# MLforHealth/LEMoN

Hardware: AMD Instinct MI355X
Metric: label-error scores/sec (embed+kNN), CIFAR-100 noise=0.4 (higher is better)
Workload: dtype f32-equivalent (fp16 x3 split GEMMs: hi.hi + hi.lo + lo.hi, fp32 accumulate, LayerNorms folded in: error <= fp32 GEMM x sqrt(1 + (mean/sigma)^2) <= 8.06, measured <= 1.8; everything else fp32)

## Files before the change

include/lemon_hip.h:

```cpp
#ifndef LEMON_HIP_H
#define LEMON_HIP_H

#include <stdint.h>

#ifdef __cplusplus
extern "C" {
#endif

#define LEMON_METRIC_IP 0
#define LEMON_METRIC_L2 1

#define LEMON_OK 0
#define LEMON_E_INVALID (-1)
#define LEMON_E_HIP (-2)
#define LEMON_E_NOMEM (-3)

#define LEMON_MAX_K 64
#define LEMON_MAX_K_DEEP 2048

#define LEMON_ALGO_AUTO 0
#define LEMON_ALGO_F32_MFMA 1
#define LEMON_ALGO_BF16_FILTER 2
#define LEMON_ALGO_F16_FILTER LEMON_ALGO_BF16_FILTER

// ... 59 lines not shown
int lemon_linear_f32(const float *x_dev, const float *w_dev, const float *bias_dev, const float *residual_dev,
                     int64_t m, int n, int k, float alpha, int act, float *y_dev, void *stream);

int lemon_linear_bf16x6(const uint16_t *x6_dev, const uint16_t *w6_dev, const float *bias_dev, const float *residual_dev,
                        int64_t m, int n, int k6, float alpha, int act, float *y_dev, void *stream);
int lemon_split3_f32(const float *x_dev, int64_t rows, int k, int weight, uint16_t *y6_dev, void *stream);
int lemon_layernorm_split3(const float *x_dev, const float *weight_dev, const float *bias_dev, float eps, int64_t rows,
                           int width, uint16_t *y6_dev, void *stream);
int lemon_linear_f16x3(const uint16_t *x3_dev, const uint16_t *w3_dev, const float *bias_dev, const float *residual_dev,
                       int64_t m, int n, int k3, float alpha, int act, float *y_dev, void *stream);
int lemon_split_f16x3(const float *x_dev, int64_t rows, int k, int weight, float wscale, uint16_t *y3_dev, void *stream);
int lemon_layernorm_f16x3(const float *x_dev, const float *weight_dev, const float *bias_dev, float eps, int64_t rows,
                          int width, uint16_t *y3_dev, void *stream);
int lemon_attention_f16x3(const float *qkv_dev, int64_t batch, int seq_len, int heads, int head_dim,
                          int causal, uint16_t *out3_dev, void *stream);
int lemon_attention_f16x3_varlen(const float *qkv_dev, int64_t batch, int seq_len, int heads, int head_dim,
                                 const int32_t *lengths_dev, uint16_t *out3_dev, void *stream);
int lemon_pack_weight_f16x3t(const float *w_dev, int n, int k, float wscale, uint16_t *wt_dev, void *stream);
int lemon_layernorm_f16x3t(const float *x_dev, const float *weight_dev, const float *bias_dev, float eps, int64_t rows,
                           int width, uint16_t *yt_dev, void *stream);
int lemon_linear_f16x3t(const uint16_t *at_dev, const uint16_t *wt_dev, const float *bias_dev, const float *residual_dev,
                        int64_t m, int n, int k, float alpha, int act, int out_operand, void *out_dev, void *stream);
int lemon_unpack_act_f16x3t(const uint16_t *at_dev, int64_t rows, int k, float *y_dev, void *stream);
int lemon_linear_f16x3t_ln(const uint16_t *at_dev, const uint16_t *wt_dev, const float *bias_dev, const float *residual_dev,
                           int64_t m, int n, int k, float alpha, int act, int out_operand, void *out_dev, const float *row_aff_dev,
                           const float *colsum_dev, uint16_t *emit_t_dev, float *emit_stats_dev, void *stream);
int lemon_linear_f16x3t_chain(const uint16_t *at_dev, const uint16_t *wt_dev, const float *bias_dev, const float *residual_dev,
                              const uint16_t *residual_t_dev, int64_t m, int n, int k, float alpha, float *out_dev,
                              uint16_t *emit_t_dev, float *emit_stats_dev, void *stream);
int lemon_ln_finalize(const float *partials_dev, int64_t rows, int width, float eps, float *row_aff_dev, void *stream);
int lemon_rowstats_f16x3t(const float *x_dev, float eps, int64_t rows, int width, uint16_t *yt_dev, float *row_aff_dev, void *stream);
int lemon_linear_f16x3t_set_profiling(int on);
int lemon_linear_f16x3t_set_mfma(int shape);
int lemon_linear_f16x3t_profile_read(int64_t *launches, double *kernel_ms, double *flops);
int lemon_attention_f16x3t(const float *qkv_dev, int64_t batch, int seq_len, int heads, int head_dim,
                           int causal, uint16_t *outt_dev, void *stream);
int lemon_attention_f16x3t_varlen(const float *qkv_dev, int64_t batch, int seq_len, int heads, int head_dim,
                                  const int32_t *lengths_dev, uint16_t *outt_dev, void *stream);
int lemon_linear_load_tuned(const char *path);
int lemon_linear_dump_tuned(const char *path);
int lemon_linear_set_tuning(int enabled);
int lemon_linear_stamp(int *hipblaslt_version, char *arch, int arch_len);


int lemon_index_create(int metric, int d, lemon_index_t **out);
int lemon_index_free(lemon_index_t *idx);

int lemon_index_add(lemon_index_t *idx, const float *x_dev, int64_t n, void *stream);

int64_t lemon_index_ntotal(const lemon_index_t *idx);
int lemon_index_dim(const lemon_index_t *idx);
const float *lemon_index_data(const lemon_index_t *idx);

int lemon_index_search(lemon_index_t *idx, const float *q_dev, int64_t nq, int k,
                       float *D_dev, int64_t *I_dev, void *stream);
int lemon_index_set_algo(lemon_index_t *idx, int algo);
int lemon_index_set_query_dedup(lemon_index_t *idx, int enabled);

typedef struct {
    int algo;
    int grid, block;
    int query_panel;
    int db_splits;
    int64_t nq, n;
    int d, k;
    int64_t nq_distinct;
// ... 94 lines not shown
```

lemon_amd/_lib.py:

```python
import ctypes
import os

_HERE = os.path.dirname(os.path.abspath(__file__))
SO_PATH = os.path.join(_HERE, "liblemon_hip.so")

METRIC_IP = 0
METRIC_L2 = 1
MAX_K = 64
MAX_K_DEEP = 2048
ATTENTION_MAX_SEQ = 4096
ALGO_AUTO, ALGO_F32_MFMA, ALGO_BF16_FILTER = 0, 1, 2

EXPORTS = [
    "lemon_last_error", "lemon_version", "lemon_normalize_rows", "lemon_paired_distance",
    "lemon_d1_normalized", "lemon_class_confidence", "lemon_paired_metric", "lemon_preprocess_u8", "lemon_preprocess_u8_f16x3t", "lemon_preprocess_ragged", "lemon_attention_f32", "lemon_attention_set_f16", "lemon_attention_set_stream_min", "lemon_attention_set_head_dims", "lemon_attention_get_head_dims", "lemon_attention_split3", "lemon_attention_f32_varlen", "lemon_attention_split3_varlen", "lemon_attention_f16x3_varlen", "lemon_attention_f16x3t_varlen", "lemon_layernorm_f32", "lemon_vision_tokens_ln", "lemon_text_tokens", "lemon_linear_f32", "lemon_linear_bf16x6", "lemon_split3_f32", "lemon_layernorm_split3", "lemon_linear_f16x3", "lemon_pack_weight_f16x3t", "lemon_layernorm_f16x3t", "lemon_linear_f16x3t", "lemon_linear_f16x3t_ln", "lemon_linear_f16x3t_chain", "lemon_ln_finalize", "lemon_rowstats_f16x3t", "lemon_unpack_act_f16x3t", "lemon_linear_f16x3t_set_profiling", "lemon_linear_f16x3t_set_mfma", "lemon_linear_f16x3t_profile_read", "lemon_attention_f16x3t", "lemon_split_f16x3", "lemon_layernorm_f16x3", "lemon_attention_f16x3", "lemon_linear_load_tuned",
    "lemon_linear_dump_tuned", "lemon_linear_set_tuning", "lemon_linear_stamp", "lemon_index_create", "lemon_index_free", "lemon_index_add",
    "lemon_index_ntotal", "lemon_index_dim", "lemon_index_data", "lemon_index_search",
    "lemon_index_set_algo", "lemon_index_set_query_dedup", "lemon_index_last_search_info", "lemon_index_set_profiling",
    "lemon_index_profile_read", "lemon_debug_scan_plan", "lemon_neighbors", "lemon_discrepancy", "lemon_score", "lemon_grid_f1",
    "lemon_kmeans_assign", "lemon_kmeans_update", "lemon_kmeans_split", "lemon_kmeans_train", "lemon_kmeans_workspace_bytes",
    "lemon_knn_label_disagreement", "lemon_jpeg_info", "lemon_jpeg_entropy", "lemon_jpeg_reconstruct_host", "lemon_jpeg_decode",
    "lemon_jpeg_pack", "lemon_jpeg_entropy_device", "lemon_jpeg_entropy_workspace_bytes", "lemon_jpeg_entropy_par_host",
    "lemon_jpeg_prog_info", "lemon_jpeg_prog_entropy", "lemon_jpeg_prog_pack", "lemon_jpeg_prog_entropy_device",
    "lemon_jpeg_prog_entropy_workspace_bytes", "lemon_jpeg_prog_entropy_par_host",
]


class LemonHipError(RuntimeError):
    pass


class SearchInfo(ctypes.Structure):
    _fields_ = [("algo", ctypes.c_int), ("grid", ctypes.c_int), ("block", ctypes.c_int),
                ("query_panel", ctypes.c_int), ("db_splits", ctypes.c_int),
                ("nq", ctypes.c_int64), ("n", ctypes.c_int64), ("d", ctypes.c_int), ("k", ctypes.c_int),
                ("nq_distinct", ctypes.c_int64)]


_lib = None


def load():
    global _lib
    if _lib is not None:
        return _lib
    if not os.path.exists(SO_PATH):
        raise LemonHipError(
            f"{SO_PATH} is missing: build it with `python -m lemon_amd.build` "
# ... 16 lines not shown
    lib.lemon_preprocess_u8_f16x3t.argtypes = [vp, c_i64, c_int, c_int, vp, vp, c_int, vp, vp, c_int, c_int, c_int, c_int,
                                        ctypes.POINTER(ctypes.c_float), ctypes.POINTER(ctypes.c_float), c_int, vp, vp]
    lib.lemon_preprocess_ragged.argtypes = [vp, c_i64, c_i64, vp, c_i64, c_i64, vp, vp, vp, c_int, ctypes.POINTER(ctypes.c_float),
                                            ctypes.POINTER(ctypes.c_float), c_int, c_int, vp, vp]
    lib.lemon_grid_f1.argtypes = [vp, vp, vp, vp, vp, vp, vp, vp, c_i64, c_int, vp, c_int, ctypes.c_double, c_int, vp, vp, vp, vp]
    lib.lemon_attention_f32.argtypes = [vp, c_i64, c_int, c_int, c_int, c_int, vp, vp]
    lib.lemon_attention_split3.argtypes = [vp, c_i64, c_int, c_int, c_int, c_int, vp, vp]
    lib.lemon_attention_f16x3.argtypes = [vp, c_i64, c_int, c_int, c_int, c_int, vp, vp]
    for name in ("f32", "split3", "f16x3", "f16x3t"):
        getattr(lib, f"lemon_attention_{name}_varlen").argtypes = [vp, c_i64, c_int, c_int, c_int, vp, vp, vp]
    lib.lemon_layernorm_f32.argtypes = [vp, vp, vp, ctypes.c_float, c_i64, c_int, vp, vp]
    lib.lemon_vision_tokens_ln.argtypes = [vp, vp, vp, vp, vp, ctypes.c_float, c_i64, c_int, c_int, vp, vp]
    lib.lemon_text_tokens.argtypes = [vp, c_i64, vp, vp, c_i64, c_int, c_int, c_int, vp, vp]
    lib.lemon_linear_f32.argtypes = [vp, vp, vp, vp, c_i64, c_int, c_int, ctypes.c_float, c_int, vp, vp]
    lib.lemon_linear_bf16x6.argtypes = [vp, vp, vp, vp, c_i64, c_int, c_int, ctypes.c_float, c_int, vp, vp]
    lib.lemon_split3_f32.argtypes = [vp, c_i64, c_int, c_int, vp, vp]
    lib.lemon_layernorm_split3.argtypes = [vp, vp, vp, ctypes.c_float, c_i64, c_int, vp, vp]
    lib.lemon_linear_f16x3.argtypes = [vp, vp, vp, vp, c_i64, c_int, c_int, ctypes.c_float, c_int, vp, vp]
    lib.lemon_split_f16x3.argtypes = [vp, c_i64, c_int, c_int, ctypes.c_float, vp, vp]
    lib.lemon_pack_weight_f16x3t.argtypes = [vp, c_int, c_int, ctypes.c_float, vp, vp]
    lib.lemon_layernorm_f16x3t.argtypes = [vp, vp, vp, ctypes.c_float, c_i64, c_int, vp, vp]
    lib.lemon_linear_f16x3t.argtypes = [vp, vp, vp, vp, c_i64, c_int, c_int, ctypes.c_float, c_int, c_int, vp, vp]
    lib.lemon_linear_f16x3t_ln.argtypes = [vp, vp, vp, vp, c_i64, c_int, c_int, ctypes.c_float, c_int, c_int, vp, vp, vp, vp, vp, vp]
    lib.lemon_linear_f16x3t_chain.argtypes = [vp, vp, vp, vp, vp, c_i64, c_int, c_int, ctypes.c_float, vp, vp, vp, vp]
    lib.lemon_ln_finalize.argtypes = [vp, c_i64, c_int, ctypes.c_float, vp, vp]
    lib.lemon_rowstats_f16x3t.argtypes = [vp, ctypes.c_float, c_i64, c_int, vp, vp, vp]
    lib.lemon_unpack_act_f16x3t.argtypes = [vp, c_i64, c_int, vp, vp]
    lib.lemon_attention_set_f16.argtypes = [c_int]
    lib.lemon_attention_set_stream_min.argtypes = [c_int]
    lib.lemon_attention_set_head_dims.argtypes = [c_int]
    lib.lemon_attention_get_head_dims.argtypes = []
    lib.lemon_linear_f16x3t_set_profiling.argtypes = [c_int]
    lib.lemon_linear_f16x3t_set_mfma.argtypes = [c_int]
    lib.lemon_linear_f16x3t_profile_read.argtypes = [ctypes.POINTER(c_i64), ctypes.POINTER(ctypes.c_double), ctypes.POINTER(ctypes.c_double)]
    lib.lemon_attention_f16x3t.argtypes = [vp, c_i64, c_int, c_int, c_int, c_int, vp, vp]
    lib.lemon_layernorm_f16x3.argtypes = [vp, vp, vp, ctypes.c_float, c_i64, c_int, vp, vp]
    lib.lemon_linear_load_tuned.argtypes = [ctypes.c_char_p]
    lib.lemon_linear_dump_tuned.argtypes = [ctypes.c_char_p]
    lib.lemon_linear_set_tuning.argtypes = [c_int]
    lib.lemon_linear_stamp.argtypes = [ctypes.POINTER(c_int), ctypes.c_char_p, c_int]
    lib.lemon_index_create.argtypes = [c_int, c_int, ctypes.POINTER(vp)]
    lib.lemon_index_free.argtypes = [vp]
    lib.lemon_index_add.argtypes = [vp, vp, c_i64, vp]
    lib.lemon_index_ntotal.argtypes = [vp]
    lib.lemon_index_ntotal.restype = c_i64
    lib.lemon_index_dim.argtypes = [vp]
    lib.lemon_index_data.argtypes = [vp]
    lib.lemon_index_data.restype = vp
    lib.lemon_index_search.argtypes = [vp, vp, c_i64, c_int, vp, vp, vp]
    lib.lemon_index_set_algo.argtypes = [vp, c_int]
    lib.lemon_index_set_query_dedup.argtypes = [vp, c_int]
    lib.lemon_index_last_search_info.argtypes = [vp, ctypes.POINTER(SearchInfo)]
    lib.lemon_index_set_profiling.argtypes = [vp, c_int]
    lib.lemon_index_profile_read.argtypes = [vp, ctypes.POINTER(c_i64)] + [ctypes.POINTER(ctypes.c_double)] * 3
    ip = ctypes.POINTER(c_int)
    lib.lemon_debug_scan_plan.argtypes = [c_int, c_int, ip, ip, ip, c_int, ip, ip, c_int, ip]
    lib.lemon_neighbors.argtypes = [vp, vp, vp, vp, vp, c_i64, c_int, c_int, vp, c_int, vp, vp] + [vp] * 9 + [vp]
    lib.lemon_discrepancy.argtypes = [c_int, vp, vp, vp, vp, c_i64, c_int, c_int, vp, vp]
    lib.lemon_score.argtypes = [vp] * 7 + [c_i64, c_int, ctypes.POINTER(ctypes.c_double), vp, vp, vp, vp]
    lib.lemon_kmeans_assign.argtypes = [vp, c_i64, c_int, vp, c_int, vp, vp, vp]
    lib.lemon_kmeans_update.argtypes = [vp, c_i64, c_int, vp, vp, c_int, vp, vp, vp, vp, c_i64, vp]
    lib.lemon_kmeans_split.argtypes = [vp, c_int, c_int, vp, vp]
    lib.lemon_kmeans_train.argtypes = [vp, c_i64, c_int, c_int, c_int, vp, vp, vp, vp, vp, c_i64, vp]
    lib.lemon_kmeans_workspace_bytes.argtypes = [c_i64, c_int, c_int]
    lib.lemon_kmeans_workspace_bytes.restype = c_i64
    lib.lemon_knn_label_disagreement.argtypes = [vp, c_i64, c_int, c_int, c_int, vp, vp, c_i64, vp, vp, vp]
# ... 25 lines not shown
```

lemon_amd/csrc/gemm_f16x3.hip:

```cpp
#include <hip/hip_runtime.h>
#include <stdint.h>
#include <cmath>
#include <cstdlib>
#include <mutex>
#include <vector>

#include "common.hpp"
#include "split3.hpp"

using namespace lemon_split;

namespace {

typedef float f32x16 __attribute__((ext_vector_type(16)));
typedef _Float16 h16x8 __attribute__((ext_vector_type(8)));
typedef _Float16 h16x4 __attribute__((ext_vector_type(4)));

constexpr int TM = TILE_A_ROWS, TN = TILE_W_ROWS;
constexpr int IB = TM / 64;
constexpr int BLKA = TM * 32, BLKW = TN * 32;
constexpr int STAGE = 2 * BLKA + 2 * BLKW;
constexpr int NB = 3, LA = NB - 1;
#ifndef LEMON_GEMM_GM
#define LEMON_GEMM_GM 32
#endif
constexpr int GM = LEMON_GEMM_GM;
constexpr int DMA_PER_STAGE = BLKA / 2048 + 4;

struct GemmParams {
    const char *at, *wt;
    const float *bias;
    const float *residual;
    void *out;
    int64_t m;
    int n, ks, m_tiles, n_tiles;
    int gm, gn;
    int vblocks;
    float alpha;
    const float2 *row_aff;
    const float *colsum;
    const unsigned short *residual_t;
    unsigned short *emit_t;
    float *emit_stats;
#ifdef LEMON_GEMM_PHASES
    unsigned long long *dbg;
#endif
};

__device__ __forceinline__ bool tile_of_workgroup(const GemmParams &p, unsigned vb, int &mt, int &nt) {
    const int xcd = vb & 7, q = vb >> 3;
    const int per = p.gm * p.gn;
    const int gm_n = (p.m_tiles + p.gm - 1) / p.gm, gn_n = (p.n_tiles + p.gn - 1) / p.gn;
    const int blk = (q / per) * 8 + xcd, pos = q % per;
    if (blk >= gm_n * gn_n) return false;
    mt = (blk / gn_n) * p.gm + pos % p.gm;
    nt = (blk % gn_n) * p.gn + pos / p.gm;
    return mt < p.m_tiles && nt < p.n_tiles;
}

__device__ __forceinline__ void mfma(f32x16 &acc, const h16x8 &a, const h16x8 &b) {
    asm volatile("v_mfma_f32_32x32x16_f16 %0, %1, %2, %0" : "+a"(acc) : "v"(a), "v"(b));
}
__device__ __forceinline__ void dma1k(const char *src, unsigned voff, unsigned lds) {
    asm volatile("s_mov_b32 m0, %2\n\ts_nop 0\n\tglobal_load_lds_dwordx4 %0, %1" : : "v"(voff), "s"(src), "s"(lds) : "memory");
}
__device__ __forceinline__ h16x8 lds128(unsigned addr, int off) {
    h16x8 v;
    asm volatile("ds_read_b128 %0, %1 offset:%2" : "=v"(v) : "v"(addr), "n"(off));
    return v;
}

template <int EPI>
__device__ __forceinline__ float epilogue_act(float u) {
    if (EPI == 2) return 0.5f * u * (1.0f + erff(u * 0.70710678118654752f));
    return u * __builtin_amdgcn_rcpf(1.0f + __expf(-u));
}
// ... 131 lines not shown
            const int n0 = nt * TN + wn * 128 + j * 32 + 4 * h;
#pragma unroll
            for (int g = 0; g < 4; ++g) {
                const int n = n0 + 8 * g;
                float4 b = make_float4(0.f, 0.f, 0.f, 0.f);
                if (p.bias) b = *reinterpret_cast<const float4 *>(p.bias + n);
                const float o[4] = {p.alpha * acc[j][i][4 * g] + b.x, p.alpha * acc[j][i][4 * g + 1] + b.y,
                                    p.alpha * acc[j][i][4 * g + 2] + b.z, p.alpha * acc[j][i][4 * g + 3] + b.w};
                h16x4 hi, lo;
#pragma unroll
                for (int e = 0; e < 4; ++e) {
                    const float v = epilogue_act<EPI>(o[e]);
                    unsigned short a_, b_, c_;
                    split2h<false>(v, a_, b_, c_);
                    hi[e] = __builtin_bit_cast(_Float16, a_); lo[e] = __builtin_bit_cast(_Float16, c_);
                }
                unsigned short *base = reinterpret_cast<unsigned short *>(p.out) + tiled_off(TM, m, n, 0, N);
                *reinterpret_cast<h16x4 *>(base) = hi;
                *reinterpret_cast<h16x4 *>(base + TM * 16) = lo;
            }
        }
    }
}

typedef float f32x4 __attribute__((ext_vector_type(4)));
__device__ __forceinline__ void mfma16(f32x4 &acc, const h16x8 &a, const h16x8 &b) {
#ifdef LEMON_MFMA16_BUILTIN
    acc = __builtin_amdgcn_mfma_f32_16x16x32_f16(a, b, acc, 0, 0, 0);
#else
    asm volatile("v_mfma_f32_16x16x32_f16 %0, %1, %2, %0" : "+a"(acc) : "v"(a), "v"(b));
#endif
}

template <int EPI, bool FOLD, bool EMIT, int LEAN = 0>
__global__ __launch_bounds__(256, 2) void k_gemm_f16x3t16(GemmParams p) {
    static_assert(!EMIT || EPI == 0, "the operand + statistics output rides on the fp32 epilogue");
    static_assert(LEAN == 0 || EMIT, "the chain options belong to the emitting form");
    extern __shared__ __attribute__((aligned(16))) char smem[];
    const int tid = threadIdx.x, lane = tid & 63, wave = __builtin_amdgcn_readfirstlane(tid >> 6);
    const int wm = wave >> 1, wn = wave & 1;
    int mt, nt;
    if (!tile_of_workgroup(p, blockIdx.x, mt, nt)) return;
#ifdef LEMON_GEMM_PHASES
    const unsigned long long ph0 = __builtin_amdgcn_s_memtime(), rt0 = __builtin_amdgcn_s_memrealtime();
    unsigned long long ph1 = 0;
#endif
    const int KS = p.ks;
    const char *a_src = p.at + (size_t)mt * KS * 2 * BLKA;
    const char *w_src = p.wt + (size_t)nt * KS * 2 * BLKW;
    const unsigned lds0 = (unsigned)(__UINTPTR_TYPE__)(__attribute__((address_space(3))) char *)smem;
    const unsigned va = (unsigned)(wave * (BLKA / 2) + lane * 16), vw = (unsigned)(wave * (BLKW / 2) + lane * 16);
    auto issue = [&](int ks, int slot) {
        const char *as = a_src + (size_t)ks * 2 * BLKA, *ws = w_src + (size_t)ks * 2 * BLKW;
        const unsigned la = lds0 + slot * STAGE + wave * (BLKA / 2), lw = lds0 + slot * STAGE + 2 * BLKA + wave * (BLKW / 2);
#pragma unroll
        for (int j = 0; j < BLKA / 2048; ++j) dma1k(as, va + j * 1024, la + j * 1024);
#pragma unroll
        for (int j = 0; j < 4; ++j) dma1k(ws, vw + j * 1024, lw + j * 1024);
    };
    f32x4 acc[8][4];
#pragma unroll
    for (int c = 0; c < 8; ++c)
#pragma unroll
        for (int b = 0; b < 4; ++b)
#pragma unroll
            for (int e = 0; e < 4; ++e) acc[c][b][e] = 0.0f;
// ... 159 lines not shown
        if (has_res) load_res(0, rn);
#define PATCH_WRITE(pass_)                                                                                       \
        do {                                                                                                     \
            float *pw_ = patch0 + ((pass_) & 1) * (32 * 36);                                                     \
            _Pragma("unroll") for (int ci = 0; ci < 2; ++ci) _Pragma("unroll") for (int bi = 0; bi < 2; ++bi) { \
                const f32x4 a = acc[2 * ((pass_) >> 1) + ci][2 * ((pass_) & 1) + bi];                            \
                *reinterpret_cast<float4 *>(pw_ + (bi * 16 + r16) * 36 + ci * 16 + 4 * kg) = make_float4(a[0], a[1], a[2], a[3]); \
            }                                                                                                    \
        } while (0)
#define EPI0_PASSES(MASKED)                                                                                      \
        _Pragma("unroll") for (int pass = 0; pass < 8; ++pass) {                                                 \
            const int cp = pass >> 1, bp = pass & 1;                                                             \
            const int n = nt * TN + wn * 128 + cp * 32 + pcol;                                                   \
            const float4 bv = bias4[cp];                                                                         \
            const int64_t m0 = (int64_t)mt * TM + wm * (IB * 32) + bp * 32;                                      \
            float4 r[4];                                                                                         \
            _Pragma("unroll") for (int q = 0; q < 4; ++q) r[q] = rn[q];                                          \
            if (has_res && pass + 1 < 8) load_res(pass + 1, rn);                                                 \
            if (pass + 1 < 8) PATCH_WRITE(pass + 1);                                                             \
            const float *pr = patch0 + (pass & 1) * (32 * 36);                                                   \
            float4 v[4];                                                                                         \
            _Pragma("unroll") for (int q = 0; q < 4; ++q) v[q] = *reinterpret_cast<const float4 *>(pr + (8 * q + prow) * 36 + pcol); \
            _Pragma("unroll") for (int q = 0; q < 4; ++q) {                                                      \
                const int64_t m = m0 + 8 * q + prow;                                                             \
                const float4 o4_ = make_float4(p.alpha * v[q].x + bv.x + r[q].x, p.alpha * v[q].y + bv.y + r[q].y, p.alpha * v[q].z + bv.z + r[q].z, p.alpha * v[q].w + bv.w + r[q].w); \
                if (!(MASKED)) *reinterpret_cast<float4 *>(out_w + (lane_off + 4u * (unsigned)((bp * 32 + 8 * q) * N + cp * 32))) = o4_; \
                else if (m < p.m) *reinterpret_cast<float4 *>(reinterpret_cast<float *>(p.out) + m * N + n) = o4_; \
            }                                                                                                    \
        }
        PATCH_WRITE(0);
        if (full) { EPI0_PASSES(false) } else { EPI0_PASSES(true) }
#undef EPI0_PASSES
#undef PATCH_WRITE
        return;
    }
    if (EPI == 0) {
        float *patch0 = reinterpret_cast<float *>(smem) + wave * (2 * 32 * 36);
        float2 *saff = reinterpret_cast<float2 *>(smem + 4 * (2 * 32 * 36) * 4) + wave * 64;
        const int prow = lane >> 3, pcol = 4 * (lane & 7);
        const bool has_res = p.residual != nullptr;
        constexpr bool res_t = (LEAN & 2) != 0;
        constexpr bool has_out = (LEAN & 1) == 0;
        const int64_t m_last = p.m - 1;
        const int64_t mw = (int64_t)mt * TM + wm * (IB * 32);
        const bool full = (int64_t)(mt + 1) * TM <= p.m;
        const int n_w = nt * TN + wn * 128;
        const int64_t wave_off = mw * N + n_w;
        const char *res_w = reinterpret_cast<const char *>(p.residual + wave_off);
        char *out_w = reinterpret_cast<char *>(reinterpret_cast<float *>(p.out) + wave_off);
        const unsigned lane_off = (unsigned)(prow * N + pcol) * 4u;
        const int64_t emit_off = 2 * ((((int64_t)mt * (N >> 4) + (n_w >> 4)) * 2) * (TM * 16) + wm * 2 * 512);
        char *emit_w = reinterpret_cast<char *>(p.emit_t) + emit_off;
        const char *rest_w = reinterpret_cast<const char *>(p.residual_t) + emit_off;
        const unsigned emit_lane = 2u * (unsigned)(((lane & 7) >> 2) * 2 * (TM * 16) + (((lane & 7) >> 1) & 1) * 256 + prow * 8 + 4 * (lane & 1));
        if (FOLD) { const int64_t m = mw + lane; saff[lane] = p.row_aff[m < m_last ? m : m_last]; }
        auto load_next = [&](int pass, float4 (&r)[4], float4 &bv, float4 &cs) {
            const int cpn = pass & 3, bpn = pass >> 2;
            const int n = n_w + cpn * 32 + pcol;
            bv = make_float4(0.f, 0.f, 0.f, 0.f); cs = bv;
            if (p.bias) bv = *reinterpret_cast<const float4 *>(p.bias + n);
            if (FOLD) cs = *reinterpret_cast<const float4 *>(p.colsum + n);
            if (res_t) {
#pragma unroll
                for (int q = 0; q < 4; ++q) {
                    const char *a_ = rest_w + (emit_lane + (unsigned)(cpn * 16384 + bpn * 1024 + q * 128));
                    const float2 h2_ = *reinterpret_cast<const float2 *>(a_), l2_ = *reinterpret_cast<const float2 *>(a_ + TM * 16 * 2);
// ... 156 lines not shown
    const int c = (int)(t - r * k);
    const float hi = f16_val(at[tiled_off(TILE_A_ROWS, r, c, 0, k)]), lo = f16_val(at[tiled_off(TILE_A_ROWS, r, c, 1, k)]);
    y[t] = hi + lo * 0.00048828125f;
}

__global__ __launch_bounds__(256) void k_ln_finalize(const float *__restrict__ part, int64_t rows, int np, float per, float eps, float2 *__restrict__ aff) {
    const int64_t r = (int64_t)blockIdx.x * blockDim.x + threadIdx.x;
    if (r >= rows) return;
    const float2 *pr = reinterpret_cast<const float2 *>(part) + r * np;
    float mean = 0.0f;
    for (int i = 0; i < np; ++i) mean += pr[i].x;
    mean /= (float)np;
    float m2 = 0.0f;
    for (int i = 0; i < np; ++i) { const float d = pr[i].x - mean; m2 += pr[i].y + per * d * d; }
    const float rstd = rsqrtf(m2 / (per * (float)np) + eps);
    const bool far = fabsf(mean) * rstd > LEMON_LN_FOLD_MAX_SHIFT;
    aff[r] = far ? make_float2(__builtin_nanf(""), __builtin_nanf("")) : make_float2(rstd, -mean * rstd);
}

constexpr int MAX_DEVICES = 64;
std::mutex g_attr_mu;
bool g_attr_set[MAX_DEVICES] = {};
struct GemmProf {
    bool on = false;
    std::vector<hipEvent_t> ev;
    std::vector<double> flops;
    size_t used = 0;
} g_prof;
constexpr size_t PROF_POOL = 2 * 1024;
int g_gm = 0, g_gn = 0;
#ifdef LEMON_GEMM_PHASES
unsigned long long *g_phase_dbg = nullptr;
#endif
int g_mfma_shape = 0;
void walk_override() {
    static bool read = false;
    if (read) return;
    read = true;
    const char *e = getenv("LEMON_GEMM_WALK");
    int a = 0, b = 0;
    if (e && sscanf(e, "%d,%d", &a, &b) == 2 && a > 0 && b > 0 && a <= 1024 && b <= 64) { g_gm = a; g_gn = b; }
}
int mfma_shape() {
    if (g_mfma_shape == 0) {
        const char *e = getenv("LEMON_GEMM_MFMA");
        g_mfma_shape = (e && atoi(e) == 32) ? 32 : 16;
    }
    return g_mfma_shape;
}

}

extern "C" int lemon_pack_weight_f16x3t(const float *w_dev, int n, int k, float wscale, uint16_t *wt_dev, void *stream_) {
    LEMON_REQUIRE(n > 0 && k > 0 && n % TN == 0 && k % 16 == 0, "n a multiple of 256, k a multiple of 16");
    LEMON_REQUIRE(w_dev && wt_dev && ((((uintptr_t)w_dev) | ((uintptr_t)wt_dev)) & 15) == 0, "aligned pointers");
    int e = 0;
    LEMON_REQUIRE(wscale > 0.0f && std::frexp(wscale, &e) == 0.5f, "wscale must be a power of two");
    const int64_t threads = (int64_t)n * (k >> 3);
    hipLaunchKernelGGL(k_pack_weight_t, dim3((unsigned)((threads + 255) / 256)), dim3(256), 0, (hipStream_t)stream_, w_dev, n, k, wscale, wt_dev);
    LEMON_HIP_CHECK(hipGetLastError());
    return LEMON_OK;
}

extern "C" int lemon_unpack_act_f16x3t(const uint16_t *at_dev, int64_t rows, int k, float *y_dev, void *stream_) {
    LEMON_REQUIRE(rows >= 0 && k > 0 && k % 16 == 0, "rows >= 0, k a multiple of 16");
    if (rows == 0) return LEMON_OK;
// ... 25 lines not shown
    return linear_f16x3t_impl(at_dev, wt_dev, bias_dev, residual_dev, m, n, k, alpha, act, out_operand, out_dev, row_aff_dev, colsum_dev, emit_t_dev, emit_stats_dev, stream_);
}

extern "C" int lemon_linear_f16x3t_chain(const uint16_t *at_dev, const uint16_t *wt_dev, const float *bias_dev, const float *residual_dev,
                                         const uint16_t *residual_t_dev, int64_t m, int n, int k, float alpha, float *out_dev,
                                         uint16_t *emit_t_dev, float *emit_stats_dev, void *stream_) {
    LEMON_REQUIRE(emit_t_dev && emit_stats_dev, "the chain form always leaves the operand and its row statistics");
    LEMON_REQUIRE(!(residual_dev && residual_t_dev), "one residual: fp32 or operand form");
    LEMON_REQUIRE(k % 32 == 0, "k a multiple of 32 (16x16x32 kernel)");
    LEMON_REQUIRE((((uintptr_t)residual_t_dev) & 15) == 0, "16-byte aligned pointers");
    return linear_f16x3t_impl(at_dev, wt_dev, bias_dev, residual_dev, m, n, k, alpha, LEMON_ACT_NONE, 0, out_dev, nullptr, nullptr, emit_t_dev,
                              emit_stats_dev, stream_, residual_t_dev);
}

static int linear_f16x3t_impl(const uint16_t *at_dev, const uint16_t *wt_dev, const float *bias_dev, const float *residual_dev,
                              int64_t m, int n, int k, float alpha, int act, int out_operand, void *out_dev,
                              const float *row_aff_dev, const float *colsum_dev, uint16_t *emit_t_dev, float *emit_stats_dev, void *stream_,
                              const uint16_t *residual_t_dev) {
    LEMON_REQUIRE(m >= 0 && n > 0 && k > 0 && n % TN == 0 && k % 16 == 0, "m >= 0, n a multiple of 256, k a multiple of 16");
    if (m == 0) return LEMON_OK;
    LEMON_REQUIRE(at_dev && wt_dev && (out_dev || emit_t_dev), "null pointer");
    LEMON_REQUIRE(((((uintptr_t)row_aff_dev) | ((uintptr_t)colsum_dev) | ((uintptr_t)emit_t_dev) | ((uintptr_t)emit_stats_dev)) & 15) == 0, "16-byte aligned pointers");
    LEMON_REQUIRE(((((uintptr_t)at_dev) | ((uintptr_t)wt_dev) | ((uintptr_t)out_dev) | ((uintptr_t)bias_dev) | ((uintptr_t)residual_dev)) & 15) == 0,
                  "16-byte aligned pointers");
    LEMON_REQUIRE((act == LEMON_ACT_NONE && !out_operand) || ((act == LEMON_ACT_SILU || act == LEMON_ACT_GELU) && out_operand && !residual_dev),
                  "supported forms: act none -> fp32 [m, n] (+ residual); act SiLU / GELU -> tile-major operand (no residual)");
    LEMON_REQUIRE((m + TM - 1) / TM < ((int64_t)1 << 24), "m < 2^31");
    GemmParams p;
    p.at = reinterpret_cast<const char *>(at_dev); p.wt = reinterpret_cast<const char *>(wt_dev);
    p.bias = bias_dev; p.residual = residual_dev; p.out = out_dev;
    p.row_aff = reinterpret_cast<const float2 *>(row_aff_dev); p.colsum = colsum_dev;
    p.emit_t = reinterpret_cast<unsigned short *>(emit_t_dev); p.emit_stats = emit_stats_dev;
    p.residual_t = reinterpret_cast<const unsigned short *>(residual_t_dev);
    p.m = m; p.n = n; p.ks = k / 16; p.m_tiles = (int)((m + TM - 1) / TM); p.n_tiles = n / TN; p.alpha = alpha;
    walk_override();
    if (g_gm > 0) { p.gm = g_gm; p.gn = g_gn > 0 ? g_gn : 1; }
    else {
        p.gn = p.n_tiles % 4 == 0 ? 4 : p.n_tiles % 3 == 0 ? 3 : p.n_tiles % 2 == 0 ? 2 : 1;
        p.gm = p.gn == 1 ? GM : p.gn == 3 ? 8 : 16;
    }
    if (p.gn > p.n_tiles) p.gn = p.n_tiles;
    const int64_t blocks = (int64_t)((p.m_tiles + p.gm - 1) / p.gm) * ((p.n_tiles + p.gn - 1) / p.gn);
    int64_t grid = ((blocks + 7) / 8) * p.gm * p.gn * 8;
    LEMON_REQUIRE(grid < ((int64_t)1 << 31), "grid size");
    p.vblocks = (int)grid;
#ifdef LEMON_GEMM_PHASES
    p.dbg = g_phase_dbg;
#endif
    const size_t lds = (size_t)NB * STAGE;
    int dev = 0;
    LEMON_HIP_CHECK(hipGetDevice(&dev));
    LEMON_REQUIRE(dev >= 0 && dev < MAX_DEVICES, "device index");
    {
        std::lock_guard<std::mutex> lock(g_attr_mu);
        if (!g_attr_set[dev]) {
            LEMON_HIP_CHECK(hipFuncSetAttribute(reinterpret_cast<const void *>(k_gemm_f16x3t<0>), hipFuncAttributeMaxDynamicSharedMemorySize, (int)lds));
            LEMON_HIP_CHECK(hipFuncSetAttribute(reinterpret_cast<const void *>(k_gemm_f16x3t<1>), hipFuncAttributeMaxDynamicSharedMemorySize, (int)lds));
            LEMON_HIP_CHECK(hipFuncSetAttribute(reinterpret_cast<const void *>(k_gemm_f16x3t16<0, false, false>), hipFuncAttributeMaxDynamicSharedMemorySize, (int)lds));
            LEMON_HIP_CHECK(hipFuncSetAttribute(reinterpret_cast<const void *>(k_gemm_f16x3t16<1, false, false>), hipFuncAttributeMaxDynamicSharedMemorySize, (int)lds));
            LEMON_HIP_CHECK(hipFuncSetAttribute(reinterpret_cast<const void *>(k_gemm_f16x3t16<0, true, false>), hipFuncAttributeMaxDynamicSharedMemorySize, (int)lds));
            LEMON_HIP_CHECK(hipFuncSetAttribute(reinterpret_cast<const void *>(k_gemm_f16x3t16<1, true, false>), hipFuncAttributeMaxDynamicSharedMemorySize, (int)lds));
            LEMON_HIP_CHECK(hipFuncSetAttribute(reinterpret_cast<const void *>(k_gemm_f16x3t16<0, false, true>), hipFuncAttributeMaxDynamicSharedMemorySize, (int)lds));
            LEMON_HIP_CHECK(hipFuncSetAttribute(reinterpret_cast<const void *>(k_gemm_f16x3t16<0, false, true, 1>), hipFuncAttributeMaxDynamicSharedMemorySize, (int)lds));
            LEMON_HIP_CHECK(hipFuncSetAttribute(reinterpret_cast<const void *>(k_gemm_f16x3t16<0, false, true, 2>), hipFuncAttributeMaxDynamicSharedMemorySize, (int)lds));
            LEMON_HIP_CHECK(hipFuncSetAttribute(reinterpret_cast<const void *>(k_gemm_f16x3t16<0, false, true, 3>), hipFuncAttributeMaxDynamicSharedMemorySize, (int)lds));
            LEMON_HIP_CHECK(hipFuncSetAttribute(reinterpret_cast<const void *>(k_gemm_f16x3t<2>), hipFuncAttributeMaxDynamicSharedMemorySize, (int)lds));
// ... 19 lines not shown
    }
    if (ev0) LEMON_HIP_CHECK(hipEventRecord(ev0, (hipStream_t)stream_));
    const bool fold = row_aff_dev != nullptr, emit = emit_t_dev != nullptr;
    const bool gelu = act == LEMON_ACT_GELU;
    if (fold || emit) {
        if (fold && out_operand && gelu) hipLaunchKernelGGL((k_gemm_f16x3t16<2, true, false>), dim3((unsigned)grid), dim3(256), lds, (hipStream_t)stream_, p);
        else if (fold && out_operand) hipLaunchKernelGGL((k_gemm_f16x3t16<1, true, false>), dim3((unsigned)grid), dim3(256), lds, (hipStream_t)stream_, p);
        else if (fold) hipLaunchKernelGGL((k_gemm_f16x3t16<0, true, false>), dim3((unsigned)grid), dim3(256), lds, (hipStream_t)stream_, p);
        else if (!residual_t_dev && out_dev) hipLaunchKernelGGL((k_gemm_f16x3t16<0, false, true>), dim3((unsigned)grid), dim3(256), lds, (hipStream_t)stream_, p);
        else if (!residual_t_dev) hipLaunchKernelGGL((k_gemm_f16x3t16<0, false, true, 1>), dim3((unsigned)grid), dim3(256), lds, (hipStream_t)stream_, p);
        else if (out_dev) hipLaunchKernelGGL((k_gemm_f16x3t16<0, false, true, 2>), dim3((unsigned)grid), dim3(256), lds, (hipStream_t)stream_, p);
        else hipLaunchKernelGGL((k_gemm_f16x3t16<0, false, true, 3>), dim3((unsigned)grid), dim3(256), lds, (hipStream_t)stream_, p);
    } else if (mf16) {
        if (out_operand && gelu) hipLaunchKernelGGL((k_gemm_f16x3t16<2, false, false>), dim3((unsigned)grid), dim3(256), lds, (hipStream_t)stream_, p);
        else if (out_operand) hipLaunchKernelGGL((k_gemm_f16x3t16<1, false, false>), dim3((unsigned)grid), dim3(256), lds, (hipStream_t)stream_, p);
        else hipLaunchKernelGGL((k_gemm_f16x3t16<0, false, false>), dim3((unsigned)grid), dim3(256), lds, (hipStream_t)stream_, p);
    } else {
        if (out_operand && gelu) hipLaunchKernelGGL(k_gemm_f16x3t<2>, dim3((unsigned)grid), dim3(256), lds, (hipStream_t)stream_, p);
        else if (out_operand) hipLaunchKernelGGL(k_gemm_f16x3t<1>, dim3((unsigned)grid), dim3(256), lds, (hipStream_t)stream_, p);
        else hipLaunchKernelGGL(k_gemm_f16x3t<0>, dim3((unsigned)grid), dim3(256), lds, (hipStream_t)stream_, p);
    }
    LEMON_HIP_CHECK(hipGetLastError());
    if (ev1) LEMON_HIP_CHECK(hipEventRecord(ev1, (hipStream_t)stream_));
    return LEMON_OK;
}

extern "C" int lemon_linear_f16x3t_set_mfma(int shape) {
    LEMON_REQUIRE(shape == 0 || shape == 16 || shape == 32, "shape: 16, 32 or 0 (the default: $LEMON_GEMM_MFMA, else 16)");
    const int prev = mfma_shape();
    g_mfma_shape = shape;
    return prev;
}

extern "C" int lemon_linear_f16x3t_set_profiling(int on) {
    std::lock_guard<std::mutex> lock(g_attr_mu);
    if (on && g_prof.ev.empty()) {
        g_prof.ev.resize(PROF_POOL);
        for (auto &e : g_prof.ev) LEMON_HIP_CHECK(hipEventCreate(&e));
    }
    g_prof.on = on != 0;
    return LEMON_OK;
}

extern "C" int lemon_linear_f16x3t_profile_read(int64_t *launches, double *kernel_ms, double *flops) {
    LEMON_REQUIRE(launches && kernel_ms && flops, "null pointer");
    std::lock_guard<std::mutex> lock(g_attr_mu);
    *launches = (int64_t)(g_prof.used / 2); *kernel_ms = 0.0; *flops = 0.0;
    for (size_t i = 0; i + 1 < g_prof.used; i += 2) {
        LEMON_HIP_CHECK(hipEventSynchronize(g_prof.ev[i + 1]));
        float ms = 0.0f;
        LEMON_HIP_CHECK(hipEventElapsedTime(&ms, g_prof.ev[i], g_prof.ev[i + 1]));
        *kernel_ms += ms; *flops += g_prof.flops[i / 2];
    }
    g_prof.used = 0; g_prof.flops.clear();
    return LEMON_OK;
}

extern "C" int lemon_ln_finalize(const float *partials_dev, int64_t rows, int width, float eps, float *row_aff_dev, void *stream_) {
    LEMON_REQUIRE(rows >= 0 && width > 0 && width % TN == 0, "rows >= 0, width a multiple of 256");
    if (rows == 0) return LEMON_OK;
    LEMON_REQUIRE(partials_dev && row_aff_dev, "null pointer");
    hipLaunchKernelGGL(k_ln_finalize, dim3((unsigned)((rows + 255) / 256)), dim3(256), 0, (hipStream_t)stream_, partials_dev, rows, width / 128, 128.0f, eps,
                       reinterpret_cast<float2 *>(row_aff_dev));
    LEMON_HIP_CHECK(hipGetLastError());
    return LEMON_OK;
}
// ... 1 lines not shown
```

lemon_amd/ops.py:

```python
import ctypes

import numpy as np
import torch

from . import _lib

_METRICS = {"cosine": _lib.METRIC_IP, "ip": _lib.METRIC_IP, "euclidean": _lib.METRIC_L2,
            "l2": _lib.METRIC_L2, _lib.METRIC_IP: _lib.METRIC_IP, _lib.METRIC_L2: _lib.METRIC_L2}


def metric_id(metric):
    try:
        return _METRICS[metric]
    except KeyError:
        raise ValueError(f"unknown metric {metric!r} (cosine|euclidean)")


def stream_ptr(device=None):
    return ctypes.c_void_p(torch.cuda.current_stream(device).cuda_stream)


def dev_f32(t, name="tensor"):
    if not torch.is_tensor(t):
        raise TypeError(f"{name}: expected a torch CUDA tensor, got {type(t).__name__}")
# ... 384 lines not shown
    if act in ("silu", "gelu"):
        assert residual is None and not emit
        out = torch.empty((_tiled_rows(m) * n * 2,), dtype=torch.float16, device=at.device)
    else:
        assert act is None
        out = torch.empty(out_shape if out_shape is not None else (m, n), dtype=torch.float32, device=at.device)
        assert out.numel() == m * n
        if residual is not None:
            assert residual.dtype == torch.float32 and residual.numel() == m * n
            residual = residual.contiguous()
    if row_aff is not None:
        assert row_aff.dtype == torch.float32 and row_aff.numel() == 2 * m and colsum.dtype == torch.float32 and colsum.numel() == n
        row_aff, colsum = row_aff.contiguous(), colsum.contiguous()
    et = st = None
    if emit:
        et = torch.empty((_tiled_rows(m) * n * 2,), dtype=torch.float16, device=at.device)
        st = torch.empty((m, n // 128, 2), dtype=torch.float32, device=at.device)
    with torch.cuda.device(at.device):
        _lib.check(lib.lemon_linear_f16x3t_ln(ptr(at), ptr(wt), ptr(bias) if bias is not None else None,
                                              ptr(residual) if residual is not None else None, m, n, k, float(alpha),
                                              _ACT_CODE[act], int(act is not None), ptr(out),
                                              ptr(row_aff) if row_aff is not None else None, ptr(colsum) if colsum is not None else None,
                                              ptr(et) if emit else None, ptr(st) if emit else None, stream_ptr(at.device)),
                   "lemon_linear_f16x3t_ln")
    return (out, et, st) if emit else out


def chain_operand_residual():
    import os
    v = os.environ.get("LEMON_CHAIN_RES", "2")
    return 0 if v == "0" else (1 if v == "1" else 2)


def linear_t_chain(at, wt, m, n, k, bias=None, residual=None, residual_t=None, alpha=1.0, out_shape=None, fp32_out=True):
    assert at.is_cuda and at.dtype == torch.float16 and wt.dtype == torch.float16
    assert at.numel() == _tiled_rows(m) * k * 2 and wt.numel() == n * k * 2 and k % 32 == 0
    assert residual is None or residual_t is None
    lib = _lib.load()
    if bias is not None:
        bias = bias.contiguous()
    out = None
    if fp32_out:
        out = torch.empty(out_shape if out_shape is not None else (m, n), dtype=torch.float32, device=at.device)
        assert out.numel() == m * n
    if residual is not None:
        assert residual.dtype == torch.float32 and residual.numel() == m * n
        residual = residual.contiguous()
    if residual_t is not None:
        assert residual_t.dtype == torch.float16 and residual_t.numel() == _tiled_rows(m) * n * 2
    et = torch.empty((_tiled_rows(m) * n * 2,), dtype=torch.float16, device=at.device)
    st = torch.empty((m, n // 128, 2), dtype=torch.float32, device=at.device)
    with torch.cuda.device(at.device):
        _lib.check(lib.lemon_linear_f16x3t_chain(ptr(at), ptr(wt), ptr(bias) if bias is not None else None,
                                                 ptr(residual) if residual is not None else None,
                                                 ptr(residual_t) if residual_t is not None else None, m, n, k, float(alpha),
                                                 ptr(out) if out is not None else None, ptr(et), ptr(st), stream_ptr(at.device)),
                   "lemon_linear_f16x3t_chain")
    return out, et, st


def gemm_profiling(on):
    _lib.check(_lib.load().lemon_linear_f16x3t_set_profiling(int(bool(on))), "lemon_linear_f16x3t_set_profiling")


def gemm_profile_read():
    n, ms, fl = ctypes.c_int64(0), ctypes.c_double(0.0), ctypes.c_double(0.0)
    _lib.check(_lib.load().lemon_linear_f16x3t_profile_read(ctypes.byref(n), ctypes.byref(ms), ctypes.byref(fl)),
               "lemon_linear_f16x3t_profile_read")
    return {"launches": int(n.value), "kernel_ms": float(ms.value), "flops": float(fl.value)}


ATTENTION_VARLEN_MAX_SEQ = 288


def attention_varlen_supported(width, heads, seq_len):
    return heads > 0 and width == 64 * heads and 1 <= seq_len <= ATTENTION_VARLEN_MAX_SEQ


def attention_lengths(lengths, batch, device):
    if torch.is_tensor(lengths) and lengths.is_cuda:
        t = lengths.to(device=device, dtype=torch.int32).contiguous()
    else:
        host = torch.as_tensor(lengths).to(torch.int32).reshape(-1).contiguous()
        t = host.pin_memory().to(device, non_blocking=True)
# ... 199 lines not shown
```

Baseline: 39070.

## Add register-direct epilogue for chained f16x3 GEMM residual path

Adds a new epilogue for the LEAN==3 chain GEMM that reads the split-fp16 residual straight from global memory with a one-step prefetch. It adds bias and residual, re-splits the result into hi/lo fp16 and writes the tiled operand directly from registers, bypassing the LDS patch staging. It also computes per-row mean/M2 statistics with in-register Welford merging and wave shuffles. This aims to cut LDS round trips and barriers in the epilogue, at the cost of uncoalesced-looking global accesses and more register pressure. It is on by default and can be switched back via an env var or a setter.

```diff
diff --git a/include/lemon_hip.h b/include/lemon_hip.h
--- a/include/lemon_hip.h
+++ b/include/lemon_hip.h
@@ -115,6 +115,7 @@
 int lemon_rowstats_f16x3t(const float *x_dev, float eps, int64_t rows, int width, uint16_t *yt_dev, float *row_aff_dev, void *stream);
 int lemon_linear_f16x3t_set_profiling(int on);
 int lemon_linear_f16x3t_set_mfma(int shape);
+int lemon_linear_f16x3t_set_chain_epi(int direct);
 int lemon_linear_f16x3t_profile_read(int64_t *launches, double *kernel_ms, double *flops);
 int lemon_attention_f16x3t(const float *qkv_dev, int64_t batch, int seq_len, int heads, int head_dim,
                            int causal, uint16_t *outt_dev, void *stream);
diff --git a/lemon_amd/_lib.py b/lemon_amd/_lib.py
--- a/lemon_amd/_lib.py
+++ b/lemon_amd/_lib.py
@@ -13,7 +13,7 @@
 
 EXPORTS = [
     "lemon_last_error", "lemon_version", "lemon_normalize_rows", "lemon_paired_distance",
-    "lemon_d1_normalized", "lemon_class_confidence", "lemon_paired_metric", "lemon_preprocess_u8", "lemon_preprocess_u8_f16x3t", "lemon_preprocess_ragged", "lemon_attention_f32", "lemon_attention_set_f16", "lemon_attention_set_stream_min", "lemon_attention_set_head_dims", "lemon_attention_get_head_dims", "lemon_attention_split3", "lemon_attention_f32_varlen", "lemon_attention_split3_varlen", "lemon_attention_f16x3_varlen", "lemon_attention_f16x3t_varlen", "lemon_layernorm_f32", "lemon_vision_tokens_ln", "lemon_text_tokens", "lemon_linear_f32", "lemon_linear_bf16x6", "lemon_split3_f32", "lemon_layernorm_split3", "lemon_linear_f16x3", "lemon_pack_weight_f16x3t", "lemon_layernorm_f16x3t", "lemon_linear_f16x3t", "lemon_linear_f16x3t_ln", "lemon_linear_f16x3t_chain", "lemon_ln_finalize", "lemon_rowstats_f16x3t", "lemon_unpack_act_f16x3t", "lemon_linear_f16x3t_set_profiling", "lemon_linear_f16x3t_set_mfma", "lemon_linear_f16x3t_profile_read", "lemon_attention_f16x3t", "lemon_split_f16x3", "lemon_layernorm_f16x3", "lemon_attention_f16x3", "lemon_linear_load_tuned",
+    "lemon_d1_normalized", "lemon_class_confidence", "lemon_paired_metric", "lemon_preprocess_u8", "lemon_preprocess_u8_f16x3t", "lemon_preprocess_ragged", "lemon_attention_f32", "lemon_attention_set_f16", "lemon_attention_set_stream_min", "lemon_attention_set_head_dims", "lemon_attention_get_head_dims", "lemon_attention_split3", "lemon_attention_f32_varlen", "lemon_attention_split3_varlen", "lemon_attention_f16x3_varlen", "lemon_attention_f16x3t_varlen", "lemon_layernorm_f32", "lemon_vision_tokens_ln", "lemon_text_tokens", "lemon_linear_f32", "lemon_linear_bf16x6", "lemon_split3_f32", "lemon_layernorm_split3", "lemon_linear_f16x3", "lemon_pack_weight_f16x3t", "lemon_layernorm_f16x3t", "lemon_linear_f16x3t", "lemon_linear_f16x3t_ln", "lemon_linear_f16x3t_chain", "lemon_ln_finalize", "lemon_rowstats_f16x3t", "lemon_unpack_act_f16x3t", "lemon_linear_f16x3t_set_profiling", "lemon_linear_f16x3t_set_mfma", "lemon_linear_f16x3t_set_chain_epi", "lemon_linear_f16x3t_profile_read", "lemon_attention_f16x3t", "lemon_split_f16x3", "lemon_layernorm_f16x3", "lemon_attention_f16x3", "lemon_linear_load_tuned",
     "lemon_linear_dump_tuned", "lemon_linear_set_tuning", "lemon_linear_stamp", "lemon_index_create", "lemon_index_free", "lemon_index_add",
     "lemon_index_ntotal", "lemon_index_dim", "lemon_index_data", "lemon_index_search",
     "lemon_index_set_algo", "lemon_index_set_query_dedup", "lemon_index_last_search_info", "lemon_index_set_profiling",
@@ -96,6 +96,7 @@
     lib.lemon_attention_get_head_dims.argtypes = []
     lib.lemon_linear_f16x3t_set_profiling.argtypes = [c_int]
     lib.lemon_linear_f16x3t_set_mfma.argtypes = [c_int]
+    lib.lemon_linear_f16x3t_set_chain_epi.argtypes = [c_int]
     lib.lemon_linear_f16x3t_profile_read.argtypes = [ctypes.POINTER(c_i64), ctypes.POINTER(ctypes.c_double), ctypes.POINTER(ctypes.c_double)]
     lib.lemon_attention_f16x3t.argtypes = [vp, c_i64, c_int, c_int, c_int, c_int, vp, vp]
     lib.lemon_layernorm_f16x3.argtypes = [vp, vp, vp, ctypes.c_float, c_i64, c_int, vp, vp]
diff --git a/lemon_amd/csrc/gemm_f16x3.hip b/lemon_amd/csrc/gemm_f16x3.hip
--- a/lemon_amd/csrc/gemm_f16x3.hip
+++ b/lemon_amd/csrc/gemm_f16x3.hip
@@ -42,6 +42,7 @@
     const unsigned short *residual_t;
     unsigned short *emit_t;
     float *emit_stats;
+    int direct;
 #ifdef LEMON_GEMM_PHASES
     unsigned long long *dbg;
 #endif
@@ -239,6 +240,104 @@
 #endif
 }
 
+constexpr int CHAIN_PF = 1;
+__device__ __forceinline__ void epilogue_chain_direct(const GemmParams &p, f32x4 (&acc)[8][4], int mt, int nt, int wm, int wn, int lane) {
+#pragma clang fp contract(off)
+    const int r16 = lane & 15, kg = lane >> 4;
+    const int N = p.n;
+    const int n_w = nt * TN + wn * 128;
+    const int64_t mw = (int64_t)mt * TM + wm * (IB * 32);
+    const int64_t wave_off = 2 * ((((int64_t)mt * (N >> 4) + (n_w >> 4)) * 2) * (TM * 16) + wm * 2 * 512);
+    char *emit_w = reinterpret_cast<char *>(p.emit_t) + wave_off;
+    const char *rest_w = reinterpret_cast<const char *>(p.residual_t) + wave_off;
+    const unsigned lane_off = 2u * (unsigned)((kg >> 1) * 256 + r16 * 8 + 4 * (kg & 1));
+    constexpr unsigned LO = TM * 16 * 2;
+    float4 rq[CHAIN_PF + 1][4], bq[CHAIN_PF + 1];
+    const bool has_bias = p.bias != nullptr;
+    typedef const __attribute__((address_space(1))) float *gfloat_p;
+    gfloat_p bias_src = (has_bias ? (gfloat_p)p.bias : (gfloat_p)p.residual_t) + n_w + 4 * kg;
+    auto fetch = [&](int c) {
+        float4 (&r)[4] = rq[c % (CHAIN_PF + 1)];
+        float4 &bv = bq[c % (CHAIN_PF + 1)];
+        const f32x4 bl = *reinterpret_cast<const __attribute__((address_space(1))) f32x4 *>(bias_src + c * 16);
+        bv = make_float4(has_bias ? bl[0] : 0.f, has_bias ? bl[1] : 0.f, has_bias ? bl[2] : 0.f, has_bias ? bl[3] : 0.f);
+#pragma unroll
+        for (int b = 0; b < 4; ++b) {
+            const char *a_ = rest_w + (lane_off + (unsigned)(c * 8192 + (b >> 1) * 1024 + (b & 1) * 256));
+            const float2 h2_ = *reinterpret_cast<const float2 *>(a_), l2_ = *reinterpret_cast<const float2 *>(a_ + LO);
+            r[b] = make_float4(h2_.x, h2_.y, l2_.x, l2_.y);
+        }
+    };
+#pragma unroll
+    for (int c = 0; c < CHAIN_PF; ++c) fetch(c);
+    float st_s[2][4], st_1[2][4], st_2[2][4];
+#pragma unroll
+    for (int c = 0; c < 8; ++c) {
+#pragma unroll
+        for (int b = 0; b < 4; ++b) asm volatile("" : "+a"(acc[c][b]));
+        if (c + CHAIN_PF < 8) fetch(c + CHAIN_PF);
+        const float4 bv = bq[c % (CHAIN_PF + 1)];
+        const float bb[4] = {bv.x, bv.y, bv.z, bv.w};
+#pragma unroll
+        for (int b = 0; b < 4; ++b) {
+            const float4 r = rq[c % (CHAIN_PF + 1)][b];
+            const h16x4 rh = __builtin_bit_cast(h16x4, make_float2(r.x, r.y)), rl = __builtin_bit_cast(h16x4, make_float2(r.z, r.w));
+            float o[4];
+            h16x4 hi, lo;
+#pragma unroll
+            for (int e = 0; e < 4; ++e) {
+                const float rr = __builtin_fmaf((float)rl[e], 0.00048828125f, (float)rh[e]);
+                o[e] = __builtin_fmaf(p.alpha, acc[c][b][e], bb[e] + rr);
+                const _Float16 hh = (_Float16)o[e];
+                hi[e] = hh; lo[e] = (_Float16)__builtin_fmaf((float)hh, -2048.0f, o[e] * 2048.0f);
+            }
+            char *base = emit_w + (lane_off + (unsigned)(c * 8192 + (b >> 1) * 1024 + (b & 1) * 256));
+            *reinterpret_cast<h16x4 *>(base) = hi;
+            *reinterpret_cast<h16x4 *>(base + LO) = lo;
+            if (c < 2) {
+                float s0 = o[0];
+                asm volatile("" : "+v"(s0));
+                st_s[c & 1][b] = s0; st_1[c & 1][b] = 0.0f; st_2[c & 1][b] = 0.0f;
+            }
+#pragma unroll
+            for (int e = 0; e < 4; ++e) {
+                const float d = o[e] - st_s[c & 1][b];
+                st_1[c & 1][b] += d; st_2[c & 1][b] = __builtin_fmaf(d, d, st_2[c & 1][b]);
+            }
+            asm volatile("" : "+v"(st_1[c & 1][b]), "+v"(st_2[c & 1][b]));
+        }
+        __builtin_amdgcn_sched_barrier(0);
+    }
+    float meanw[4], m2w[4];
+#pragma unroll
+    for (int b = 0; b < 4; ++b) {
+        float mean[2], m2[2];
+#pragma unroll
+        for (int h = 0; h < 2; ++h) {
+            mean[h] = __builtin_fmaf(st_1[h][b], 0.0625f, st_s[h][b]);
+            m2[h] = __builtin_fmaf(st_1[h][b] * st_1[h][b], -0.0625f, st_2[h][b]);
+            float cnt = 16.0f;
+#pragma unroll
+            for (int off = 16; off < 64; off <<= 1) {
+                const float mo = __shfl_xor(mean[h], off), m2o = __shfl_xor(m2[h], off);
+                const float dm = mo - mean[h];
+                m2[h] = __builtin_fmaf(dm * dm, 0.5f * cnt, m2[h] + m2o);
+                mean[h] = 0.5f * (mean[h] + mo);
+                cnt *= 2.0f;
+            }
+        }
+        const float dm = mean[1] - mean[0];
+        m2w[b] = __builtin_fmaf(dm * dm, 32.0f, m2[0] + m2[1]);
+        meanw[b] = 0.5f * (mean[0] + mean[1]);
+    }
+#pragma unroll
+    for (int b = 0; b < 4; ++b) {
+        const int64_t m = mw + b * 16 + r16;
+        if (kg == 0 && m < p.m)
+            *reinterpret_cast<float2 *>(p.emit_stats + (m * (2 * p.n_tiles) + 2 * nt + wn) * 2) = make_float2(meanw[b], m2w[b]);
+    }
+}
+
 template <int EPI, bool FOLD, bool EMIT, int LEAN = 0>
 __global__ __launch_bounds__(256, 2) void k_gemm_f16x3t16(GemmParams p) {
     static_assert(!EMIT || EPI == 0, "the operand + statistics output rides on the fp32 epilogue");
@@ -464,6 +563,10 @@
         if (full) { EPI0_PASSES(false) } else { EPI0_PASSES(true) }
 #undef EPI0_PASSES
 #undef PATCH_WRITE
+        return;
+    }
+    if (LEAN == 3 && p.direct) {
+        epilogue_chain_direct(p, acc, mt, nt, wm, wn, lane);
         return;
     }
     if (EPI == 0) {
@@ -686,6 +789,7 @@
 #ifdef LEMON_GEMM_PHASES
 unsigned long long *g_phase_dbg = nullptr;
 #endif
+int g_chain_direct = 1;
 int g_mfma_shape = 0;
 void walk_override() {
     static bool read = false;
@@ -777,6 +881,7 @@
     p.row_aff = reinterpret_cast<const float2 *>(row_aff_dev); p.colsum = colsum_dev;
     p.emit_t = reinterpret_cast<unsigned short *>(emit_t_dev); p.emit_stats = emit_stats_dev;
     p.residual_t = reinterpret_cast<const unsigned short *>(residual_t_dev);
+    p.direct = g_chain_direct;
     p.m = m; p.n = n; p.ks = k / 16; p.m_tiles = (int)((m + TM - 1) / TM); p.n_tiles = n / TN; p.alpha = alpha;
     walk_override();
     if (g_gm > 0) { p.gm = g_gm; p.gn = g_gn > 0 ? g_gn : 1; }
@@ -862,6 +967,13 @@
     return prev;
 }
 
+extern "C" int lemon_linear_f16x3t_set_chain_epi(int direct) {
+    LEMON_REQUIRE(direct == 0 || direct == 1, "direct: 1 (register-direct epilogue) or 0 (LDS patches)");
+    const int prev = g_chain_direct;
+    g_chain_direct = direct;
+    return prev;
+}
+
 extern "C" int lemon_linear_f16x3t_set_profiling(int on) {
     std::lock_guard<std::mutex> lock(g_attr_mu);
     if (on && g_prof.ev.empty()) {
diff --git a/lemon_amd/ops.py b/lemon_amd/ops.py
--- a/lemon_amd/ops.py
+++ b/lemon_amd/ops.py
@@ -440,6 +440,44 @@
     return 0 if v == "0" else (1 if v == "1" else 2)
 
 
+_forced_chain_epi = None
+_chain_epi_applied = None
+
+
+class chain_epilogue_forced:
+
+    def __init__(self, mode):
+        assert mode in ("direct", "patch")
+        self.mode = mode
+
+    def __enter__(self):
+        global _forced_chain_epi
+        self.prev, _forced_chain_epi = _forced_chain_epi, self.mode
+        return self
+
+    def __exit__(self, *exc):
+        global _forced_chain_epi
+        _forced_chain_epi = self.prev
+        return False
+
+
+def chain_epilogue():
+    import os
+    v = (_forced_chain_epi or os.environ.get("LEMON_CHAIN_EPI", "direct")).lower()
+    if v not in ("direct", "patch"):
+        raise ValueError(f"LEMON_CHAIN_EPI={v!r}: direct or patch")
+    return v
+
+
+def _apply_chain_epilogue(lib):
+    global _chain_epi_applied
+    v = chain_epilogue()
+    if v != _chain_epi_applied:
+        if lib.lemon_linear_f16x3t_set_chain_epi(int(v == "direct")) < 0:
+            _lib.check(-1, "lemon_linear_f16x3t_set_chain_epi")
+        _chain_epi_applied = v
+
+
 def linear_t_chain(at, wt, m, n, k, bias=None, residual=None, residual_t=None, alpha=1.0, out_shape=None, fp32_out=True):
     assert at.is_cuda and at.dtype == torch.float16 and wt.dtype == torch.float16
     assert at.numel() == _tiled_rows(m) * k * 2 and wt.numel() == n * k * 2 and k % 32 == 0
@@ -458,6 +496,7 @@
         assert residual_t.dtype == torch.float16 and residual_t.numel() == _tiled_rows(m) * n * 2
     et = torch.empty((_tiled_rows(m) * n * 2,), dtype=torch.float16, device=at.device)
     st = torch.empty((m, n // 128, 2), dtype=torch.float32, device=at.device)
+    _apply_chain_epilogue(lib)
     with torch.cuda.device(at.device):
         _lib.check(lib.lemon_linear_f16x3t_chain(ptr(at), ptr(wt), ptr(bias) if bias is not None else None,
                                                  ptr(residual) if residual is not None else None,
```

Measured after the change: 39240, median of 6. No clear change (+0.4%).
